# rongzhao-zhang/EfficientQ

Measured on AMD Instinct MI355X. Metric: ptq_calibration_throughput, higher is better.
Workload: dtype i8xi8->i32 (exact) for the Gram systems and per-iteration loss convs of the layers with quantised input, f32/f64 elsewhere

## Files before the change

### efficientq_amd/_lib.py

```python
from __future__ import annotations

import ctypes as C
import os

import torch

_HERE = os.path.dirname(os.path.abspath(__file__))
LIB_PATH = os.path.join(_HERE, "libeffq_hip.so")

EFFQ_OK = 0
_ERR_NAMES = {1: "EFFQ_ERR_ARG", 2: "EFFQ_ERR_HIP", 3: "EFFQ_ERR_WORKSPACE", 4: "EFFQ_ERR_NO_DEVICE",
              5: "EFFQ_ERR_NOT_CONVERGED"}


class EffqError(RuntimeError):
    pass


class Geom(C.Structure):
    _fields_ = [(n, C.c_int32) for n in
                ("N", "C1", "C2", "D", "H", "W", "KD", "KH", "KW", "SD", "SH", "SW", "PD", "PH", "PW")]

    def out_dims(self):
        return ((self.D + 2 * self.PD - self.KD) // self.SD + 1,
# ... 52 lines not shown
    "effq_quant_dequant_f64path": (_I, [_P, _P, _D, _D, _I, _P, _P, _P, _SZ, _P]),
    "effq_reduce_ws_bytes": (_SZ, []),
    "effq_abs_sum_f64": (_I, [_P, _SZ, _P, _P, _P]),
    "effq_moments_f64": (_I, [_P, _SZ, _P, _P, _P]),
    "effq_alpha_stats_f64": (_I, [_P, _P, _D, _D, _I, _SZ, _P, _P, _P, _P]),
    "effq_fp_init": (_I, [_P, _P, _P]),
    "effq_fp_update": (_I, [_P, _D, _I, _P]),
    "effq_alpha_fixed_point": (_I, [_P, _SZ, _I, _D, _D, _D, _I, _I, _P, _P, _P]),
    "effq_fp_small_max": (_SZ, []),
    "effq_fixed_point_small": (_I, [_P, _P, _P, _SZ, _I, _D, _D, _D, _I, _P, _P]),
    "effq_fp_coop_max": (_SZ, []),
    "effq_fp_coop_set_spin_limit": (_I, [C.c_uint]),
    "effq_fixed_point_coop": (_I, [_P, _P, _P, _SZ, _I, _D, _D, _D, _I, _P, _P, _P]),
    "effq_fp_bucket_max": (_SZ, []),
    "effq_fp_bucket_ws_bytes": (_SZ, [_SZ]),
    "effq_fixed_point_bucket": (_I, [_P, _P, _P, _SZ, _I, _D, _D, _D, _I, _P, _P, _SZ, _P]),
    "effq_fp_bracket_ws_bytes": (_SZ, [_SZ]),
    "effq_fp_bracket_init": (_I, [_P, _P, _SZ, _I, _I, _P, _SZ, _P]),
    "effq_fp_bracket_run": (_I, [_P, _SZ, _I, _D, _D, _D, _I, _I, _P, _P, _P]),
    "effq_fp_bracket_stats": (_I, [_P, _SZ, _I, _D, _D, _P, _P, _P]),
    "effq_fp_bracket_update": (_I, [_SZ, _I, _D, _D, _D, _I, _P, _P, _P]),
    "effq_fp_traj_max": (_SZ, []),
    "effq_fp_traj_ws_bytes": (_SZ, [_SZ]),
    "effq_spd_inverse_prepare": (_I, [_P]),
    "effq_fp_traj_pred_bytes": (_SZ, []),
    "effq_fixed_point_traj": (_I, [_P, _P, _P, _SZ, _I, _D, _D, _D, _I, _P, _P, _P, _SZ, _P]),
    "effq_fixed_point_bucket_rec": (_I, [_P, _P, _P, _SZ, _I, _D, _D, _D, _I, _P, _P, _SZ, _P, _P]),
    "effq_fixed_point_coop_rec": (_I, [_P, _P, _P, _SZ, _I, _D, _D, _D, _I, _P, _P, _P, _P]),
    "effq_fp_check": (_I, [_P, _P, _P]),
    "effq_fp_channels_max_row": (_I, []),
    "effq_fixed_point_channels": (_I, [_P, _P, _P, _I, _I, _I, _D, _I, _P, _P, _P, _P]),
    "effq_fixed_point_channels_proj": (_I, [_P, _P, _P, _I, _I, _I, _D, _I, _P, _P, _P, _P, _F, _P, _P, _P, _I, _I, _D,
                                            _D, _P]),
    "effq_gram_packed_elems": (_SZ, [_I, _I]),
    "effq_gram_pack": (_I, [_P, _P, _I, _I, _P, _P]),
    "effq_gram_unpack": (_I, [_P, _I, _I, _P, _P, _P]),
    "effq_act_quant_backward": (_I, [_P, _P, _I, _P, _P, _P, _SZ, _P, _P]),
    "effq_att_classes_ws_bytes": (_SZ, []),
    "effq_att_classes": (_I, [_P, _LL, _P, _P, _P, C.POINTER(C.c_int32), _P, _P]),
    "effq_prof_enable": (_I, [_I]),
    "effq_prof_count": (_I, []),
    "effq_prof_read": (_I, [_I, C.POINTER(ProfRecord)]),
    "effq_admm_num_inverses": (_I, [_D, _D, _I, _I]),
    "effq_admm_run": (_I, [C.POINTER(AdmmRunArgs)]),
    "effq_admm_select_best": (_I, [_P, _I, _P, _P, _SZ, _SZ, _P, _P, _P, _P]),
    "effq_gram_ws_bytes": (_SZ, [_GP, _I]),
    "effq_gram_accum": (_I, [_P, _P, _P, _GP, _I, _P, _P, _I, _P, _SZ, _P]),
    "effq_gram_plan_query": (_I, [_GP, _I, _IP, _IP, _IP, _IP, _LLP, _IP, _IP]),
    "effq_gram_i8_supported": (_I, [_GP, _I]),
    "effq_gram_i8_ws_bytes": (_SZ, [_GP, _I]),
    "effq_gram_accum_i8": (_I, [_P, _P, _GP, _I, _P, _I, _P, _P, _P, _I, _LL, _P, _P, _I, _P, _SZ, _P]),
    "effq_gram_accum_i8_unw": (_I, [_P, _P, _GP, _I, _P, _I, _P, _P, _P, _I, _LL, _P, _P, _I, _P, _P, _P, _SZ, _P]),
    "effq_gram_i8_plan_query": (_I, [_GP, _I, _LL, _IP, _IP, _IP, _IP, _IP, _IP]),
    "effq_upsample_trilinear": (_I, [_P, _I, _I, _I, _I, _I, _I, _I, _I, _P, _P]),
    "effq_gram_f64_supported": (_I, [_GP, _I]),
    "effq_gram_f64_ws_bytes": (_SZ, [_GP, _I]),
    "effq_gram_f64": (_I, [_P, _P, _GP, _I, _P, _P, _P, _SZ, _P]),
    "effq_gram_f64_plan_query": (_I, [_GP, _I, _IP, _IP, _IP, _IP]),
    "effq_gram_f64_pipelined": (_I, [_P, _P, _GP, _I]),
    "effq_gram_loss_ws_bytes": (_SZ, [_I]),
    "effq_gram_loss": (_I, [_P, _P, _P, _P, _P, _I, _I, _I, _P, _P, _SZ, _P]),
    "effq_packed_bytes": (_SZ, [_SZ, _I]),
    "effq_pack_levels": (_I, [_P, _SZ, _I, _P, _P]),
    "effq_unpack_levels": (_I, [_P, _SZ, _I, _P, _P]),
    "effq_ainv_ld": (_I, [_I]),
    "effq_fp_bracket_export_words": (_SZ, []),
    "effq_fp_bracket_export": (_I, [_P, _SZ, _P, _P, _SZ, _P]),
    "effq_fp_bracket_rebase": (_I, [_P, _P, _SZ, _P]),
    "effq_fp_bracket_import": (_I, [_P, _SZ, _P, _I, _SZ, _P, _P, _SZ, _P]),
    "effq_admm_uses_traj": (_I, [_SZ, _I]),
    "effq_gram_loss_i8_supported": (_I, [_I, _I, _I, _I]),
    "effq_gram_loss_i8_num_planes": (_I, [C.c_longlong]),
    "effq_gram_loss_i8_planes_bytes": (_SZ, [_I, _I, _I]),
    "effq_gram_loss_i8_prepare": (_I, [_P, _I, _I, _P, _I, _I, _P, _P, _P]),
    "effq_gram_loss_i8_ws_bytes": (_SZ, []),
    "effq_gram_loss_i8": (_I, [_P, _I, _P, _P, _P, _P, _P, _P, _P, _I, _I, _I, _I, _I, _I, _P, _P, _SZ, _P]),
    "effq_spd_inverse_ws_bytes": (_SZ, [_I]),
    "effq_spd_inverse": (_I, [_P, _I, _I, _D, _D, _P, _P, _SZ, _P]),
    "effq_spd_inverse_plan": (_I, [_I, _IP, _IP, _IP]),
    "effq_prox_plan_query": (_I, [_I, _I, _IP, _IP, _IP, _IP]),
    "effq_prox_ws_bytes": (_SZ, [_I, _I]),
    "effq_prox_solve": (_I, [_P, _P, _P, _P, _P, _P, _I, _I, _I, _D, _D, _P, _P, _P, _SZ, _P]),
    "effq_prox_solve_shifted": (_I, [_P, _P, _P, _P, _P, _P, _I, _I, _I, _D, _D, _D, _I, _P, _P, _P, _SZ, _P]),
    "effq_admm_presum": (_I, [_P, _P, _P, _SZ, _P]),
    "effq_admm_project_dual": (_I, [_P, _P, _P, _I, _P, _P, _F, _P, _SZ, _P]),
    "effq_conv_plan_query": (_I, [_GP, _I, _IP, _IP, _IP, _IP, _IP, _IP, _IP, _IP, _LLP]),
    "effq_conv_i8_plan_query": (_I, [_GP, _I, _IP, _IP, _IP, _IP]),
    "effq_conv_i8s_plan_query": (_I, [_GP, _I, _I, _IP, _IP, _IP, _IP, _IP, _IP, _IP]),
    "effq_conv_i8_supported": (_I, [_GP, _I, _I]),
    "effq_conv_i8s_supported": (_I, [_GP, _I, _I]),
    "effq_conv_i8s_ws_bytes": (_SZ, [_GP, _I, _I]),
    "conv3d_calib_step_i8s": (_I, [_P, _P, _P, _P, _GP, _P, _I, _P, _I, _I, _P, _P, _SZ, _P]),
    "effq_conv_i8_ws_bytes": (_SZ, [_GP]),
    "conv3d_calib_step_i8": (_I, [_P, _P, _P, _P, _GP, _P, _I, _P, _I, _P, _P, _SZ, _P]),
    "effq_conv_i8_out_supported": (_I, [_GP, _I, _I]),
    "conv3d_quant_forward_i8": (_I, [_P, _P, _P, _P, _P, _GP, _P, _I, _P, _I, _P, _P, _P, _SZ, _P]),
    "effq_conv_ws_bytes": (_SZ, [_GP]),
    "conv3d_quant_calib_step": (_I, [_P, _P, _P, _P, _P, _GP, _P, _I, _P, _P, _P, _SZ, _P]),
    "effq_adam_step": (_I, [_P, _P, _P, _P, _D, _D, _D, _D, _I, _SZ, _P]),
    "effq_window_gather": (_I, [_P, _I, _I, _I, _I, _I, _I, _I, _I, _I, _I, _I, _I, _I, _I, _P, _P]),
    "effq_window_put": (_I, [_P, _I, _I, _I, _I, _I, _I, _I, _P, _P]),
    "effq_window_stitch": (_I, [_P, _I, _I, _I, _I, _I, _I, _I, _I, _I, _I, _I, _P, _P, _P, _I, _P, _P]),
    "effq_seg_tallies": (_I, [_P, _P, _I, _LL, _I, _I, _F, _P, _P, _SZ, _P]),
    "effq_seg_sweep": (_I, [_P, _P, _I, _LL, _I, _I, _F, _P, _P]),
    "effq_seg_sweep_edges": (_I, [_I, _F, _P]),
    "effq_seg_sweep_plan": (_I, [_I, _LL, _I, _IP, _IP]),
# ... 73 lines not shown
```

### efficientq_amd/csrc/gram_i8.hip

```cpp
#include <stdint.h>
#include <stdlib.h>
#include "common.h"

namespace effq {

typedef int gi_v4i __attribute__((ext_vector_type(4)));
typedef int gi_v16i __attribute__((ext_vector_type(16)));

constexpr int GI_KC = 128;
constexpr int GI_MB = 128;
constexpr int GI_RS = GI_KC + 16;
constexpr int GI_T = 256;
constexpr int GI_PANEL = GI_MB * GI_RS;
constexpr int GI_LDS = 4 * GI_PANEL + 2 * GI_KC * 16;
constexpr int GI_MAXCLS = 16;
constexpr int GI_MAX_CPS = 1000;

struct GramI8Params {
  const uint8_t* x;
  const int8_t* yd;
  const int* vox_list;
  const int* chunk_cls;
  const int* vtab;
  int N, C1, C2, C2P, D, H, W, OD, OH, OW;
  int KD, KH, KW, SD, SH, SW, PD, PH, PW;
  int T, RX, YR0, E, NB, NBX, npairs;
  long long V;
  int nchunks, nsplit, cps, ncls;
  long long* slabs;
  int debug;
};

__device__ __forceinline__ void gi_transpose4(int r0, int r1, int r2, int r3, int (&o)[4]) {
  const int t0 = __builtin_amdgcn_perm(r1, r0, 0x05010400);
  const int t1 = __builtin_amdgcn_perm(r1, r0, 0x07030602);
  const int t2 = __builtin_amdgcn_perm(r3, r2, 0x05010400);
  const int t3 = __builtin_amdgcn_perm(r3, r2, 0x07030602);
  o[0] = __builtin_amdgcn_perm(t2, t0, 0x05040100);
  o[1] = __builtin_amdgcn_perm(t2, t0, 0x07060302);
  o[2] = __builtin_amdgcn_perm(t3, t1, 0x05040100);
  o[3] = __builtin_amdgcn_perm(t3, t1, 0x07060302);
}

__device__ __forceinline__ gi_v4i gi_build_entry(const GramI8Params& p, int v) {
  gi_v4i e = {0, 0, 0, 0};
  if (v < 0) return e;
  int t = v;
  const int ow = t % p.OW;
  t /= p.OW;
  const int oh = t % p.OH;
  t /= p.OH;
  const int od = t % p.OD;
  const int n = t / p.OD;
  const int id0 = od * p.SD - p.PD, ih0 = oh * p.SH - p.PH, iw0 = ow * p.SW - p.PW;
  unsigned m = 0x80000000u;
  int tap = 0;
  for (int kd = 0; kd < p.KD; ++kd)
    for (int kh = 0; kh < p.KH; ++kh)
      for (int kw = 0; kw < p.KW; ++kw, ++tap) {
        const int id = id0 + kd, ih = ih0 + kh, iw = iw0 + kw;
        const bool ok = id >= 0 && id < p.D && ih >= 0 && ih < p.H && iw >= 0 && iw < p.W;
        m |= (ok ? 1u : 0u) << tap;
      }
  e[0] = ((n * p.D + id0) * p.H + ih0) * p.W + iw0;
  e[1] = (int)m;
  e[2] = v;
  return e;
}

__global__ __launch_bounds__(256) void k_gi_voxtable(GramI8Params p, gi_v4i* __restrict__ table) {
  const long long nslots = (long long)p.nchunks * GI_KC;
  const long long stride = (long long)gridDim.x * blockDim.x;
  for (long long s = (long long)blockIdx.x * blockDim.x + threadIdx.x; s < nslots; s += stride) {
    const int v = (p.vox_list != nullptr) ? p.vox_list[s] : ((s < p.V) ? (int)s : -1);
    table[s] = gi_build_entry(p, v);
  }
}

__global__ __launch_bounds__(GI_T, 2) void k_gram_i8(GramI8Params p) {
  extern __shared__ __attribute__((aligned(16))) unsigned char gi_smem[];
  unsigned char* const panI = gi_smem;
  unsigned char* const panJ = gi_smem + 2 * GI_PANEL;
  gi_v4i* const tbl = reinterpret_cast<gi_v4i*>(gi_smem + 4 * GI_PANEL);

  const int tid = threadIdx.x, lane = tid & 63, wid = tid >> 6;
  const int li = lane & 31, lh = lane >> 5;
  const int wr = wid >> 1, wc = wid & 1;

  int I = 0, rem = blockIdx.x;
  while (rem >= p.NB - I) {
    rem -= p.NB - I;
    ++I;
  }
  const int J = I + rem;
  const bool diag = (I == J);

  const int c_begin = blockIdx.y * p.cps;
  const int c_end = min(c_begin + p.cps, p.nchunks);
  if (c_begin >= c_end) return;

  const int vg = tid & 31, rg = tid >> 5;
  int kindI, tapI, offI, kindJ, tapJ, offJ;
  auto make_rg = [&](int r0, int& kind, int& tap, int& off) {
    kind = 3;
    tap = 0;
    off = 0;
    if (r0 < p.RX) {
      kind = 0;
      tap = r0 / p.C1;
      const int c0 = r0 - tap * p.C1;
      const int kw = tap % p.KW, t2 = tap / p.KW;
      const int kh = t2 % p.KH, kd = t2 / p.KH;
      off = ((kd * p.H + kh) * p.W + kw) * p.C1 + c0;
    } else if (r0 == p.RX) {
      kind = 2;
    } else if (r0 >= p.YR0 && r0 < p.E) {
      kind = 1;
      off = r0 - p.YR0;
    }
  };
  make_rg(I * GI_MB + 16 * rg, kindI, tapI, offI);
  make_rg(J * GI_MB + 16 * rg, kindJ, tapJ, offJ);
  const unsigned char* const srcI = (kindI == 1) ? reinterpret_cast<const unsigned char*>(p.yd) : p.x;
  const unsigned char* const srcJ = (kindJ == 1) ? reinterpret_cast<const unsigned char*>(p.yd) : p.x;
  const int ystride = 4 * p.C2P;

  const gi_v4i* const vtab = reinterpret_cast<const gi_v4i*>(p.vtab);

  gi_v4i vI[4], vJ[4];
  unsigned okI = 0, okJ = 0;
#define GI_FETCH(val, okb, kind, tap, off, src, slot)                                            \
  {                                                                                              \
    okb = 0;                                                                                     \
    _Pragma("unroll") for (int q = 0; q < 4; ++q) {                                              \
      const gi_v4i e = tbl[(slot) * GI_KC + vg + 32 * q];                                        \
      const unsigned m = (unsigned)e[1];                                                         \
      const unsigned okx = (m >> (tap)) & 1u, okv = m >> 31;                                     \
      const unsigned ok = (kind == 0) ? okx : ((kind <= 2) ? okv : 0u);                          \
      const int ax = okx ? (e[0] * p.C1 + (off)) : 0;                                            \
      const int ay = e[2] * ystride + (off);                                                     \
      const int addr = (kind == 0) ? ax : ((kind == 1) ? ay : 0);                                \
      val[q] = *reinterpret_cast<const gi_v4i*>(src + ((EFFQ_DBG(p) == 2) ? 0 : addr));             \
      okb |= ok << q;                                                                            \
    }                                                                                            \
  }
  auto stage = [&](unsigned char* P, gi_v4i (&val)[4], unsigned okb, int kind) {
#pragma unroll
    for (int q = 0; q < 4; ++q) {
      const bool ok = (okb >> q) & 1u;
      gi_v4i z = {0, 0, 0, 0};
      if (kind == 2) z[0] = 1;
      if (!ok || kind >= 2) val[q] = ok ? z : gi_v4i{0, 0, 0, 0};
    }
#pragma unroll
    for (int k = 0; k < 4; ++k) {
      int o[4];
      gi_transpose4(val[0][k], val[1][k], val[2][k], val[3][k], o);
#pragma unroll
      for (int b = 0; b < 4; ++b) *reinterpret_cast<int*>(P + (16 * rg + 4 * k + b) * GI_RS + 4 * vg) = o[b];
    }
  };

  gi_v16i acc[2][2];
#pragma unroll
  for (int m = 0; m < 2; ++m)
#pragma unroll
    for (int n = 0; n < 2; ++n)
#pragma unroll
      for (int r = 0; r < 16; ++r) acc[m][n][r] = 0;
  const bool live = (I * GI_MB + wr * 64 < p.E) && (J * GI_MB + wc * 64 < p.E);

  auto flush = [&](int cls) {
    long long* S = p.slabs + ((size_t)cls * p.npairs + blockIdx.x) * (size_t)(GI_MB * GI_MB);
#pragma unroll
    for (int m = 0; m < 2; ++m)
#pragma unroll
      for (int n = 0; n < 2; ++n)
#pragma unroll
        for (int r = 0; r < 16; ++r) {
          const int row = wr * 64 + m * 32 + (r & 3) + 8 * (r >> 2) + 4 * lh;
          const int col = wc * 64 + n * 32 + li;
          const int v = acc[m][n][r];
          if (v != 0)
            atomicAdd(reinterpret_cast<unsigned long long*>(&S[row * GI_MB + col]), (unsigned long long)(long long)v);
          acc[m][n][r] = 0;
        }
  };

  {
    const int k = tid & (GI_KC - 1);
    const int cc = (tid < GI_KC) ? c_begin : min(c_begin + 1, c_end - 1);
    tbl[(tid < GI_KC ? 0 : 1) * GI_KC + k] = vtab[(size_t)cc * GI_KC + k];
  }
  __syncthreads();
  GI_FETCH(vI, okI, kindI, tapI, offI, srcI, 0)
  if (!diag) GI_FETCH(vJ, okJ, kindJ, tapJ, offJ, srcJ, 0)
  stage(panI, vI, okI, kindI);
  if (!diag) stage(panJ, vJ, okJ, kindJ);
  __syncthreads();

  const bool has_cls = p.chunk_cls != nullptr;
  const int* const clsp = has_cls ? p.chunk_cls : reinterpret_cast<const int*>(p.x);
  int cls_cur = has_cls ? clsp[c_begin] : 0;
  int cls_next = (c_begin + 1 < c_end) ? (has_cls ? clsp[c_begin + 1] : 0) : -1;
  for (int c = c_begin; c < c_end; ++c) {
    const int b = (c - c_begin) & 1;
    const int c2 = min(c + 2, c_end - 1);
    const int cls_raw = clsp[has_cls ? c2 : 0];
    const gi_v4i traw = vtab[(size_t)c2 * GI_KC + (tid & (GI_KC - 1))];
    GI_FETCH(vI, okI, kindI, tapI, offI, srcI, b ^ 1)
    if (!diag) GI_FETCH(vJ, okJ, kindJ, tapJ, offJ, srcJ, b ^ 1)
    __builtin_amdgcn_sched_barrier(0);
    if (live && EFFQ_DBG(p) != 1) {
      const unsigned char* PI = panI + b * GI_PANEL + (wr * 64 + li) * GI_RS + lh * 16;
      const unsigned char* PJ = (diag ? panI : panJ) + b * GI_PANEL + (wc * 64 + li) * GI_RS + lh * 16;
#pragma unroll
      for (int s = 0; s < GI_KC / 32; ++s) {
        gi_v4i a[2], bb[2];
#pragma unroll
        for (int m = 0; m < 2; ++m) a[m] = *reinterpret_cast<const gi_v4i*>(PI + m * 32 * GI_RS + s * 32);
#pragma unroll
        for (int n = 0; n < 2; ++n) bb[n] = *reinterpret_cast<const gi_v4i*>(PJ + n * 32 * GI_RS + s * 32);
#pragma unroll
        for (int m = 0; m < 2; ++m)
#pragma unroll
          for (int n = 0; n < 2; ++n) acc[m][n] = __builtin_amdgcn_mfma_i32_32x32x32_i8(a[m], bb[n], acc[m][n], 0, 0, 0);
      }
    }
    if (cls_next != cls_cur && live) flush(cls_cur);
    if (tid < GI_KC) tbl[b * GI_KC + tid] = traw;
    if (EFFQ_DBG(p) != 3) {
      stage(panI + (b ^ 1) * GI_PANEL, vI, okI, kindI);
      if (!diag) stage(panJ + (b ^ 1) * GI_PANEL, vJ, okJ, kindJ);
    }
    cls_cur = cls_next;
    cls_next = (c + 2 < c_end) ? (has_cls ? cls_raw : 0) : -1;
    __syncthreads();
  }
#undef GI_FETCH
}

__global__ __launch_bounds__(256) void k_gi_absmax(const float* __restrict__ y, size_t n, unsigned* __restrict__ out) {
  float m = 0.0f;
  const size_t stride = (size_t)gridDim.x * blockDim.x;
  for (size_t e = (size_t)blockIdx.x * blockDim.x + threadIdx.x; e < n; e += stride) m = fmaxf(m, fabsf(y[e]));
#pragma unroll
  for (int o = 32; o > 0; o >>= 1) m = fmaxf(m, __shfl_xor(m, o));
  if ((threadIdx.x & 63) == 0) atomicMax(out, __float_as_uint(m));
}

__device__ __forceinline__ int gi_y_exponent(unsigned ymax_bits) {
  const float ymax = __uint_as_float(ymax_bits);
  int ex = 0;
  if (ymax > 0.0f && ymax < 3.0e38f) (void)frexpf(ymax, &ex);
  return ex < -90 ? -90 : ex;
}

__global__ __launch_bounds__(256) void k_gi_ydigits(const float* __restrict__ y, long long V, int C2, int C2P,
                                                    const unsigned* __restrict__ ymax_bits, int8_t* __restrict__ yd) {
  const int ex = gi_y_exponent(*ymax_bits);
  const float scale = ldexpf(1.0f, 30 - ex);
  const size_t tot = (size_t)V * C2P, stride = (size_t)gridDim.x * blockDim.x;
  for (size_t e = (size_t)blockIdx.x * blockDim.x + threadIdx.x; e < tot; e += stride) {
    const size_t v = e / C2P;
    const int c = (int)(e - v * C2P);
    int d[4] = {0, 0, 0, 0};
    if (c < C2) {
      float f = y[v * C2 + c] * scale;
      if (!(fabsf(f) < 1.1e9f)) f = 0.0f;
      int t = (int)rintf(f);
#pragma unroll
      for (int k = 0; k < 3; ++k) {
        d[k] = ((t + 128) & 255) - 128;
        t = (t - d[k]) >> 8;
      }
      d[3] = t;
    }
    int8_t* dst = yd + v * (size_t)(4 * C2P) + c;
#pragma unroll
    for (int k = 0; k < 4; ++k) dst[(size_t)k * C2P] = (int8_t)d[k];
  }
}

__global__ __launch_bounds__(256) void k_gram_i8_finish(GramI8Params p, int n, int hb, const float* __restrict__ alpha,
                                                        int act_levels, const unsigned* __restrict__ ymax_bits,
                                                        const float* __restrict__ cls_w, float* __restrict__ A0,
// ... 56 lines not shown
      }
      val = 2.0 * q * (xb ? s : 1.0) * t;
      dst = B0 + f;
      if (Bu != nullptr) {
        const double vu = q * (xb ? s : 1.0) * tu;
        Bu[f] = accumulate ? Bu[f] + vu : vu;
      }
    }
    *dst = accumulate ? (*dst + (float)val) : (float)val;
  }
}

static int gram_i8_plan(const effq_geom* g, int ncls, long long n_list, GramI8Params* pp) {
  EFFQ_CHECK_ARG(g != nullptr);
  EFFQ_CHECK_ARG(g->N > 0 && g->C1 > 0 && g->C2 > 0 && g->D > 0 && g->H > 0 && g->W > 0);
  EFFQ_CHECK_ARG(g->KD >= 1 && g->KH >= 1 && g->KW >= 1 && g->SD >= 1 && g->SH >= 1 && g->SW >= 1);
  EFFQ_CHECK_ARG((g->C1 % 16) == 0 && g->KD * g->KH * g->KW <= 31);
  EFFQ_CHECK_ARG(ncls >= 1 && ncls <= GI_MAXCLS);
  GramI8Params& p = *pp;
  memset(&p, 0, sizeof(p));
  p.N = g->N; p.C1 = g->C1; p.C2 = g->C2; p.D = g->D; p.H = g->H; p.W = g->W;
  p.KD = g->KD; p.KH = g->KH; p.KW = g->KW; p.SD = g->SD; p.SH = g->SH; p.SW = g->SW;
  p.PD = g->PD; p.PH = g->PH; p.PW = g->PW;
  p.OD = (g->D + 2 * g->PD - g->KD) / g->SD + 1;
  p.OH = (g->H + 2 * g->PH - g->KH) / g->SH + 1;
  p.OW = (g->W + 2 * g->PW - g->KW) / g->SW + 1;
  EFFQ_CHECK_ARG(p.OD > 0 && p.OH > 0 && p.OW > 0);
  p.C2P = (g->C2 + 15) / 16 * 16;
  p.T = p.KD * p.KH * p.KW;
  p.RX = p.T * p.C1;
  p.YR0 = p.RX + 16;
  p.E = p.YR0 + 4 * p.C2P;
  p.NB = (p.E + GI_MB - 1) / GI_MB;
  p.NBX = (p.YR0 + GI_MB - 1) / GI_MB;
  p.npairs = p.NBX * p.NB - p.NBX * (p.NBX - 1) / 2;
  p.V = (long long)p.N * p.OD * p.OH * p.OW;
  EFFQ_CHECK_ARG((long long)g->N * g->D * g->H * g->W * g->C1 < (1ll << 31));
  EFFQ_CHECK_ARG(p.V * 4 * p.C2P < (1ll << 31));
  const long long nchunks = (n_list > 0) ? n_list / GI_KC : (p.V + GI_KC - 1) / GI_KC;
  EFFQ_CHECK_ARG(nchunks > 0 && nchunks < (1ll << 24));
  p.nchunks = (int)nchunks;
  p.ncls = ncls;
  long long want = (3072 + p.npairs - 1) / p.npairs;
  if (want > nchunks / 4) want = nchunks / 4;
  if (want < 1) want = 1;
  long long cps = (nchunks + want - 1) / want;
  if (cps > GI_MAX_CPS) cps = GI_MAX_CPS;
  p.cps = (int)cps;
  p.nsplit = (int)((nchunks + cps - 1) / cps);
  EFFQ_CHECK_ARG(p.nsplit <= 65535);
  return EFFQ_OK;
}

static size_t gram_i8_table_bytes(long long V, int ncls) { return (size_t)(V + (long long)GI_KC * (ncls + 1)) * 16; }

static size_t gram_i8_slab_bytes(const GramI8Params& p) {
  return (size_t)p.ncls * p.npairs * (size_t)(GI_MB * GI_MB) * sizeof(long long);
}

}

using namespace effq;

extern "C" {

int effq_gram_i8_supported(const effq_geom* g, int act_levels) {
  if (g == nullptr) return 0;
  if ((g->C1 % 16) != 0 || g->KD * g->KH * g->KW > 31 || g->KD < 1 || g->KH < 1 || g->KW < 1) return 0;
  if (act_levels < 2 || act_levels > 128) return 0;
  GramI8Params p;
  if (gram_i8_plan(g, 1, 0, &p) != EFFQ_OK) return 0;
  return 1;
}

size_t effq_gram_i8_ws_bytes(const effq_geom* g, int ncls) {
  GramI8Params p;
  if (gram_i8_plan(g, ncls, 0, &p) != EFFQ_OK) return 0;
  return 256 + gram_i8_slab_bytes(p) + (size_t)p.V * 4 * p.C2P + 256 + gram_i8_table_bytes(p.V, ncls) + 256;
}

int effq_gram_accum_i8_unw(const uint8_t* xidx_ndhwc, const float* y_ndhwc, const effq_geom* g, int has_bias,
                           const float* act_alpha_dev, int act_levels, const int32_t* vox_list, const int32_t* chunk_cls,
                           const float* cls_w_dev, int ncls, long long n_list, float* A0, float* B0, int accumulate,
                           double* Au, double* Bu, void* ws, size_t ws_bytes, void* stream) {
  EFFQ_CHECK_ARG((Au == nullptr) == (Bu == nullptr));
  EFFQ_CHECK_ARG(xidx_ndhwc && y_ndhwc && g && act_alpha_dev && A0 && B0 && ws);
  EFFQ_CHECK_ARG(effq_gram_i8_supported(g, act_levels));
  if (vox_list == nullptr) {
    EFFQ_CHECK_ARG(ncls == 1 && chunk_cls == nullptr && n_list == 0);
  } else {
    EFFQ_CHECK_ARG(chunk_cls != nullptr && cls_w_dev != nullptr && n_list > 0 && (n_list % GI_KC) == 0);
  }
  GramI8Params p;
  int rc = gram_i8_plan(g, ncls, n_list, &p);
  if (rc != EFFQ_OK) return rc;
  const size_t slab_bytes = gram_i8_slab_bytes(p);
  const size_t need = 256 + slab_bytes + (size_t)p.V * 4 * p.C2P + 256 + gram_i8_table_bytes(p.V, ncls) + 256;
  EFFQ_CHECK_ARG((size_t)p.nchunks * GI_KC * 16 <= gram_i8_table_bytes(p.V, ncls));
  if (ws_bytes < need) {
    set_error("gram_i8: workspace %zu < required %zu", ws_bytes, need);
    return EFFQ_ERR_WORKSPACE;
  }
  char* base = reinterpret_cast<char*>(ws);
  unsigned* ymax = reinterpret_cast<unsigned*>(base);
  p.slabs = reinterpret_cast<long long*>(base + 256);
  int8_t* yd = reinterpret_cast<int8_t*>(base + 256 + slab_bytes);
  gi_v4i* vtab = reinterpret_cast<gi_v4i*>((reinterpret_cast<uintptr_t>(base + 256 + slab_bytes + (size_t)p.V * 4 * p.C2P) + 255) & ~(uintptr_t)255);
  p.x = xidx_ndhwc;
  p.yd = yd;
  p.vox_list = vox_list;
  p.chunk_cls = chunk_cls;
  p.vtab = reinterpret_cast<const int*>(vtab);
  p.debug = effq_ablate_env("EFFQ_GI8_DEBUG");
  hipStream_t st = as_stream(stream);
  EFFQ_HIP(hipMemsetAsync(base, 0, 256 + slab_bytes, st));
  const size_t ny = (size_t)p.V * p.C2;
  {
    size_t nb = (ny + 255) / 256;
    if (nb > 2048) nb = 2048;
    hipLaunchKernelGGL(k_gi_absmax, dim3((unsigned)nb), dim3(256), 0, st, y_ndhwc, ny, ymax);
    size_t nd = ((size_t)p.V * p.C2P + 255) / 256;
    if (nd > 8192) nd = 8192;
    hipLaunchKernelGGL(k_gi_ydigits, dim3((unsigned)nd), dim3(256), 0, st, y_ndhwc, p.V, p.C2, p.C2P, ymax, yd);
    EFFQ_LAUNCH_CHECK();
  }
  {
    size_t nt = ((size_t)p.nchunks * GI_KC + 255) / 256;
    if (nt > 4096) nt = 4096;
    hipLaunchKernelGGL(k_gi_voxtable, dim3((unsigned)nt), dim3(256), 0, st, p, vtab);
    EFFQ_LAUNCH_CHECK();
  }
  EFFQ_HIP(raise_lds_limit<k_gram_i8>(GI_LDS));
  hipLaunchKernelGGL(k_gram_i8, dim3((unsigned)p.npairs, (unsigned)p.nsplit), dim3(GI_T), GI_LDS, st, p);
  EFFQ_LAUNCH_CHECK();
  const int n = p.RX + (has_bias ? 1 : 0);
  size_t tot = (size_t)n * n + (size_t)p.C2 * n;
  size_t nb = (tot + 255) / 256;
  if (nb > 8192) nb = 8192;
  hipLaunchKernelGGL(k_gram_i8_finish, dim3((unsigned)nb), dim3(256), 0, st, p, n, has_bias ? 1 : 0, act_alpha_dev,
                     act_levels, ymax, cls_w_dev, A0, B0, accumulate, Au, Bu);
  EFFQ_LAUNCH_CHECK();
  return EFFQ_OK;
}

int effq_gram_i8_plan_query(const effq_geom* g, int ncls, long long n_list, int* nb, int* nbx, int* npairs, int* nchunks,
                            int* cps, int* nsplit) {
  EFFQ_CHECK_ARG(nb && nbx && npairs && nchunks && cps && nsplit && n_list >= 0 && (n_list % GI_KC) == 0);
  GramI8Params p;
  const int rc = gram_i8_plan(g, ncls, n_list, &p);
  if (rc != EFFQ_OK) return rc;
  *nb = p.NB;
  *nbx = p.NBX;
  *npairs = p.npairs;
  *nchunks = p.nchunks;
  *cps = p.cps;
  *nsplit = p.nsplit;
  return EFFQ_OK;
}

int effq_gram_accum_i8(const uint8_t* xidx_ndhwc, const float* y_ndhwc, const effq_geom* g, int has_bias,
                       const float* act_alpha_dev, int act_levels, const int32_t* vox_list, const int32_t* chunk_cls,
                       const float* cls_w_dev, int ncls, long long n_list, float* A0, float* B0, int accumulate,
                       void* ws, size_t ws_bytes, void* stream) {
  return effq_gram_accum_i8_unw(xidx_ndhwc, y_ndhwc, g, has_bias, act_alpha_dev, act_levels, vox_list, chunk_cls,
                                cls_w_dev, ncls, n_list, A0, B0, accumulate, nullptr, nullptr, ws, ws_bytes, stream);
}

}

namespace effq {
constexpr int CLS_SLOTS = 32;
constexpr int CLS_MAX = 16;
struct ClsTable {
  unsigned key[CLS_SLOTS];
  unsigned cnt[CLS_SLOTS];
  unsigned cursor[CLS_MAX];
  int overflow;
  int ncls;
  int n_list;
  int slot_cls[CLS_SLOTS];
  unsigned seg_start[CLS_MAX];
  float cls_w[CLS_MAX];
};

__device__ __forceinline__ int cls_find_or_insert(unsigned* keys, unsigned k) {
  unsigned h = (k * 2654435761u) >> 27;
  for (int probe = 0; probe < CLS_SLOTS; ++probe) {
    const unsigned cur = atomicCAS(&keys[h], 0xffffffffu, k);
    if (cur == 0xffffffffu || cur == k) return (int)h;
    h = (h + 1) & (CLS_SLOTS - 1);
  }
  return -1;
}

__global__ __launch_bounds__(256) void k_cls_count(const float* __restrict__ att, long long V, ClsTable* t) {
  __shared__ unsigned lkey[CLS_SLOTS], lcnt[CLS_SLOTS];
  __shared__ int lover;
  if (threadIdx.x < CLS_SLOTS) {
    lkey[threadIdx.x] = 0xffffffffu;
    lcnt[threadIdx.x] = 0u;
  }
  if (threadIdx.x == 0) lover = 0;
  __syncthreads();
  const long long stride = (long long)gridDim.x * blockDim.x;
  for (long long i = (long long)blockIdx.x * blockDim.x + threadIdx.x; i < V; i += stride) {
    const unsigned k = __float_as_uint(att[i]);
    const int sidx = (k == 0xffffffffu) ? -1 : cls_find_or_insert(lkey, k);
    if (sidx < 0)
      lover = 1;
// ... 112 lines not shown
```

### efficientq_amd/hip_ops.py

```python
from __future__ import annotations

import ctypes as C
import math
from typing import Optional, Tuple

import torch

from . import _lib
from ._lib import Geom, check

ADMM_TOL = 1e-5
FP_BRACKET_MIN = 1 << 18
DP_GATHER_AFTER = 4
DP_GATHER_MAX_BYTES = 128 << 20


def _ptr(t: Optional[torch.Tensor]):
    return None if t is None else C.c_void_p(t.data_ptr())


def to_ndhwc(x: torch.Tensor) -> torch.Tensor:
    return x.permute(0, 2, 3, 4, 1).contiguous()


# ... 337 lines not shown
                                                 100 * levels, _ptr(state), _ptr(self._red_ws), _ptr(pred), self.stream),
              "effq_fixed_point_coop_rec")

    @staticmethod
    def read_fp_pred(pred: torch.Tensor):
        i32 = pred[:16].view(torch.int32).cpu()
        f = pred[16:16 + 8 * 40].view(torch.float64).cpu()
        i64 = pred[16 + 8 * 40:16 + 8 * 45].view(torch.int64).cpu()
        fn = pred[16 + 8 * 45:16 + 8 * 53].view(torch.float64).cpu()
        j64 = pred[16 + 8 * 53:16 + 8 * 63].view(torch.int64).cpu()
        K = int(i32[0])
        return {"K": K, "e": int(i32[1]), "lo": f[0:8].tolist(), "hi": f[8:16].tolist(), "eps": f[16:24].tolist(),
                "eps_n": fn.tolist(), "calls": int(i64[0]), "warm_iters": int(i64[1]), "full_iters": int(i64[2]),
                "listed": int(i64[3]), "list_max": int(i64[4]), "ring_iters": int(j64[0]), "ring_listed": int(j64[1]),
                "trace_us": [(int(j64[2 + k]) - int(j64[2])) / 100.0 for k in range(5)],
                "mean_us_phase1_setup_loop": [int(j64[7 + k]) / 100.0 / max(int(i64[0]), 1) for k in range(3)]}

    def fp_check(self, state, err_flag):
        check(self.lib.effq_fp_check(_ptr(state), _ptr(err_flag), self.stream), "effq_fp_check")

    def gram(self, x_ndhwc: torch.Tensor, att: Optional[torch.Tensor], y_ndhwc: torch.Tensor, geom: Geom,
             has_bias: bool, A0: Optional[torch.Tensor] = None, B0: Optional[torch.Tensor] = None):
        x = self._f32(x_ndhwc)
        y = self._f32(y_ndhwc)
        a = self._f32(att) if att is not None else None
        _check_shapes(geom, x, y=y, att=a)
        n = geom.C1 * geom.KD * geom.KH * geom.KW + int(has_bias)
        acc = int(A0 is not None)
        if A0 is not None and (tuple(A0.shape) != (n, n) or tuple(B0.shape) != (geom.C2, n)):
            raise _lib.EffqError("gram: A0/B0 shapes do not match the geometry")
        if A0 is None:
            A0 = torch.empty(n, n, dtype=torch.float32, device=self.device)
            B0 = torch.empty(geom.C2, n, dtype=torch.float32, device=self.device)
        need = self.lib.effq_gram_ws_bytes(C.byref(geom), int(has_bias))
        ws = self._workspace("gram", need)
        check(self.lib.effq_gram_accum(_ptr(x), _ptr(a), _ptr(y), C.byref(geom), int(has_bias), _ptr(A0), _ptr(B0),
                                       acc, _ptr(ws), ws.numel(), self.stream), "effq_gram_accum")
        return A0, B0

    def gram_plan(self, geom: Geom, has_bias: bool) -> dict:
        vec, nb, npairs, nsplit, fold, fin = (C.c_int() for _ in range(6))
        vps = C.c_longlong()
        check(self.lib.effq_gram_plan_query(C.byref(geom), int(has_bias), C.byref(vec), C.byref(nb), C.byref(npairs),
                                            C.byref(nsplit), C.byref(vps), C.byref(fold), C.byref(fin)),
              "effq_gram_plan_query")
        return dict(vec=bool(vec.value), NB=nb.value, npairs=npairs.value, nsplit=nsplit.value, vox_per_split=vps.value,
                    fold=fold.value, finish_blocks=fin.value)

    def gram_i8_plan(self, geom: Geom, ncls: int = 1, n_list: int = 0) -> dict:
        out = [C.c_int() for _ in range(6)]
        check(self.lib.effq_gram_i8_plan_query(C.byref(geom), int(ncls), int(n_list), *[C.byref(o) for o in out]),
              "effq_gram_i8_plan_query")
        return dict(zip(("NB", "NBX", "npairs", "nchunks", "cps", "nsplit"), (o.value for o in out)))

    def gram_f64_plan(self, geom: Geom, has_bias: bool) -> dict:
        out = [C.c_int() for _ in range(4)]
        check(self.lib.effq_gram_f64_plan_query(C.byref(geom), int(has_bias), *[C.byref(o) for o in out]),
              "effq_gram_f64_plan_query")
        return dict(zip(("nchunk", "grid", "ntiles", "tpw"), (o.value for o in out)))

    def gram_i8_supported(self, geom: Geom, act_levels: int) -> bool:
        return bool(self.lib.effq_gram_i8_supported(C.byref(geom), int(act_levels)))

    GRAM_I8_MAX_CLASSES = 16

    def att_classes(self, att: Optional[torch.Tensor]):
        if att is None:
            return (None, None, None, 1)
        key = (att.data_ptr(), att.numel(), att._version)
        hit = self._att_cache.get(key)
        if hit is not None:
            return hit[1]
        flat = self._f32(att).reshape(-1)
        V = flat.numel()
        lst = torch.empty(V + 128 * self.GRAM_I8_MAX_CLASSES, dtype=torch.int32, device=flat.device)
        chunk_cls = torch.empty(V // 128 + self.GRAM_I8_MAX_CLASSES, dtype=torch.int32, device=flat.device)
        cls_w = torch.empty(self.GRAM_I8_MAX_CLASSES, dtype=torch.float32, device=flat.device)
        info = (C.c_int32 * 3)()
        ws = self._workspace("att_cls", self.lib.effq_att_classes_ws_bytes())
        check(self.lib.effq_att_classes(_ptr(flat), V, _ptr(lst), _ptr(chunk_cls), _ptr(cls_w), info, _ptr(ws),
                                        self.stream), "effq_att_classes")
        k, n_list, overflow = int(info[0]), int(info[1]), int(info[2])
        res = None if overflow else (lst[:n_list], chunk_cls[: n_list // 128], cls_w[:k], k)
        if len(self._att_cache) > 16:
            self._att_cache.clear()
        self._att_cache[key] = (att, res)
        return res

    def gram_i8(self, xidx_ndhwc: torch.Tensor, att_cls, y_ndhwc: torch.Tensor, geom: Geom, has_bias: bool,
                act_alpha: torch.Tensor, act_levels: int, A0: Optional[torch.Tensor] = None,
                B0: Optional[torch.Tensor] = None, unweighted: bool = False):
        if xidx_ndhwc.dtype != torch.uint8 or not xidx_ndhwc.is_contiguous():
            raise _lib.EffqError("gram_i8 wants contiguous uint8 level ids")
        y = self._f32(y_ndhwc)
        _check_shapes(geom, xidx_ndhwc, y=y)
        lst, chunk_cls, cls_w, ncls = att_cls
        if lst is not None:
            od, oh, ow = geom.out_dims()
            if (int(lst.numel()) < geom.N * od * oh * ow or lst.numel() % 128 or
                    chunk_cls.numel() * 128 != lst.numel() or cls_w.numel() != ncls):
                raise _lib.EffqError("gram_i8: voxel list does not match the output volume")
        n = geom.C1 * geom.KD * geom.KH * geom.KW + int(has_bias)
        acc = int(A0 is not None)
        if A0 is not None and (tuple(A0.shape) != (n, n) or tuple(B0.shape) != (geom.C2, n)):
            raise _lib.EffqError("gram_i8: A0/B0 shapes do not match the geometry")
        if A0 is None:
# ... 1105 lines not shown
```

### include/effq_hip.h

```cpp
#ifndef EFFQ_HIP_H
#define EFFQ_HIP_H

#include <stddef.h>
#include <stdint.h>

#ifdef __cplusplus
extern "C" {
#endif

enum {
  EFFQ_OK = 0,
  EFFQ_ERR_ARG = 1,
  EFFQ_ERR_HIP = 2,
  EFFQ_ERR_WORKSPACE = 3,
  EFFQ_ERR_NO_DEVICE = 4,
  EFFQ_ERR_NOT_CONVERGED = 5
};

typedef struct effq_geom {
  int32_t N, C1, C2;
  int32_t D, H, W;
  int32_t KD, KH, KW;
  int32_t SD, SH, SW;
  int32_t PD, PH, PW;
// ... 50 lines not shown
size_t effq_fp_traj_pred_bytes(void);
int effq_fixed_point_traj(const float* a, const float* b, float* v_out, size_t n, int levels, double lo, double hi,
                          double tol, int max_iter, effq_fp_state* state_dev, void* pred_dev, void* ws, size_t ws_bytes,
                          void* stream);
int effq_fixed_point_bucket_rec(const float* a, const float* b, float* v_out, size_t n, int levels, double lo, double hi,
                                double tol, int max_iter, effq_fp_state* state_dev, void* ws, size_t ws_bytes,
                                void* pred_dev, void* stream);
int effq_fixed_point_coop_rec(const float* a, const float* b, float* v_out, size_t n, int levels, double lo, double hi,
                              double tol, int max_iter, effq_fp_state* state_dev, void* ws, void* pred_dev, void* stream);

size_t effq_fp_bracket_ws_bytes(size_t n);
int effq_fp_bracket_init(effq_fp_state* state_dev, const double* abs_sums_dev, size_t n, int levels, int list_first,
                         void* ws, size_t ws_bytes, void* stream);
int effq_fp_bracket_run(const float* x, size_t n, int levels, double lo, double hi, double tol, int max_iter, int n_iters,
                        effq_fp_state* state_dev, void* ws, void* stream);
int effq_fp_bracket_stats(const float* x, size_t n, int levels, double lo, double hi, effq_fp_state* state_dev, void* ws,
                          void* stream);
int effq_fp_bracket_update(size_t n, int levels, double lo, double hi, double tol, int max_iter,
                           effq_fp_state* state_dev, void* ws, void* stream);
size_t effq_fp_bracket_export_words(void);
int effq_fp_bracket_export(const void* ws, size_t n, long long* out, float* list_out, size_t list_cap, void* stream);
int effq_fp_bracket_import(const void* ws_src, size_t n_src, const long long* pack_dev, int world, size_t list_cap,
                           effq_fp_state* state_dev, void* ws_dst, size_t ws_dst_bytes, void* stream);
int effq_fp_bracket_rebase(effq_fp_state* state_dev, void* ws, size_t n, void* stream);
int effq_fp_channels_max_row(void);
int effq_fixed_point_channels(const float* a, const float* b, float* v_out, int c2, int nwrow, int levels, double tol,
                              int max_iter, double* alpha_out, int32_t* iters_out, int32_t* err_flag_dev, void* stream);
int effq_fixed_point_channels_proj(const float* wstar, float* dual, float* v_out, int c2, int nwrow, int levels,
                                   double tol, int max_iter, double* alpha_out, int32_t* iters_out, int32_t* err_flag_dev,
                                   float* G, float dual_div, float* Bm, const float* B0, const float* W0, int n, int ldb,
                                   double rho_next, double eta, void* stream);

int effq_fp_check(const effq_fp_state* state_dev, int32_t* err_flag_dev, void* stream);

size_t effq_gram_ws_bytes(const effq_geom* g, int has_bias);
int effq_gram_accum(const float* x_ndhwc, const float* att, const float* y_ndhwc, const effq_geom* g,
                    int has_bias, float* A0, float* B0, int accumulate, void* ws, size_t ws_bytes,
                    void* stream);
int effq_gram_plan_query(const effq_geom* g, int has_bias, int* vec, int* nb, int* npairs, int* nsplit,
                         long long* vox_per_split, int* fold, int* finish_blocks);

int effq_gram_i8_supported(const effq_geom* g, int act_levels);
size_t effq_gram_i8_ws_bytes(const effq_geom* g, int ncls);
int effq_gram_accum_i8(const uint8_t* xidx_ndhwc, const float* y_ndhwc, const effq_geom* g, int has_bias,
                       const float* act_alpha_dev, int act_levels, const int32_t* vox_list,
                       const int32_t* chunk_cls, const float* cls_w_dev, int ncls, long long n_list,
                       float* A0, float* B0, int accumulate, void* ws, size_t ws_bytes, void* stream);
int effq_gram_accum_i8_unw(const uint8_t* xidx_ndhwc, const float* y_ndhwc, const effq_geom* g, int has_bias,
                           const float* act_alpha_dev, int act_levels, const int32_t* vox_list, const int32_t* chunk_cls,
                           const float* cls_w_dev, int ncls, long long n_list, float* A0, float* B0, int accumulate,
                           double* Au, double* Bu, void* ws, size_t ws_bytes, void* stream);
int effq_gram_i8_plan_query(const effq_geom* g, int ncls, long long n_list, int* nb, int* nbx, int* npairs, int* nchunks,
                            int* cps, int* nsplit);

int effq_gram_f64_supported(const effq_geom* g, int has_bias);
size_t effq_gram_f64_ws_bytes(const effq_geom* g, int has_bias);
int effq_gram_f64(const float* x_ndhwc, const float* y_ndhwc, const effq_geom* g, int has_bias, double* Au, double* Bu,
                  void* ws, size_t ws_bytes, void* stream);
int effq_gram_f64_plan_query(const effq_geom* g, int has_bias, int* nchunk, int* grid, int* ntiles, int* tpw);
int effq_gram_f64_pipelined(const float* x_ndhwc, const float* y_ndhwc, const effq_geom* g, int has_bias);

size_t effq_gram_loss_ws_bytes(int n);
int effq_gram_loss(const double* Au, const double* Bu, const double* syy_dev, const float* G, const float* b, int c2, int n,
                   int has_bias, double* sqerr_out, void* ws, size_t ws_bytes, void* stream);

int effq_gram_loss_i8_supported(int c2, int n, int has_bias, int w_levels);
int effq_gram_loss_i8_num_planes(long long kmax);
size_t effq_gram_loss_i8_planes_bytes(int n, int has_bias, int nplanes);
int effq_gram_loss_i8_prepare(const double* Au, int n, int has_bias, const float* act_alpha_dev, int act_levels,
                              int nplanes, int8_t* planes, int32_t* err_flag_dev, void* stream);
size_t effq_gram_loss_i8_ws_bytes(void);
int effq_gram_loss_i8(const int8_t* planes, int nplanes, const double* Au, const double* Bu, const double* syy_dev,
                      const int8_t* Gq, const float* b, const effq_fp_state* states, const float* act_alpha_dev,
                      int act_levels, int w_levels, int c2, int n, int has_bias, int count, double* hist_out, void* ws,
                      size_t ws_bytes, void* stream);


size_t effq_att_classes_ws_bytes(void);
int effq_att_classes(const float* att, long long V, int32_t* vox_list, int32_t* chunk_cls, float* cls_w_dev,
                     int32_t* info_host_out, void* ws, void* stream);

int effq_spd_inverse_prepare(void* stream);
int effq_ainv_ld(int n);
size_t effq_spd_inverse_ws_bytes(int n);
int effq_spd_inverse(const float* A0, int n, int has_bias, double rho, double eta, float* Ainv,
                     void* ws, size_t ws_bytes, void* stream);
int effq_spd_inverse_plan(int n, int* wide, int* nblk, int* pivot_blocks);

size_t effq_prox_ws_bytes(int c2, int n);
int effq_prox_solve(const float* B0, const float* Ainv, const float* W0, const float* b0, const float* G,
                    const float* dual, int c2, int n, int has_bias, double rho, double eta, float* wstar,
                    float* bstar, void* ws, size_t ws_bytes, void* stream);
int effq_prox_plan_query(int c2, int n, int* variant, int* gx, int* gy, int* nsplit);

int effq_prox_solve_shifted(const float* B0, const float* Ainv, const float* W0, const float* b0, const float* G,
                            const float* dual, int c2, int n, int has_bias, double rho, double eta,
                            double rho_inv, int nterms, float* wstar, float* bstar, void* ws, size_t ws_bytes,
                            void* stream);

int effq_admm_presum(const float* wstar, const float* dual, float* v, size_t n, void* stream);
int effq_admm_project_dual(const float* v, const float* wstar, const effq_fp_state* state_dev, int levels,
                           float* G, float* dual, float dual_div, int8_t* Gq_out, size_t n, void* stream);
size_t effq_conv_ws_bytes(const effq_geom* g);
int conv3d_quant_calib_step(const float* xq_ndhwc, const float* G, const float* bias, const float* y_fp,
                            const float* att, const effq_geom* g, const float* act_alpha_dev, int act_levels,
                            double* sqerr_out, float* out, void* ws, size_t ws_bytes, void* stream);
// ... 186 lines not shown
```

Baseline: 25.23.

## Group 2x2 Gram tile pairs per block and sub-split chunk ranges

The int8 Gram kernel is templated on a group size G. With G=2, one 512-thread block computes a 2x2 group of 128x128 tile pairs, and each wave holds a 128x64 accumulator. Every staged I/J panel now feeds two output tiles instead of one, roughly halving global gathers and LDS staging per MFMA. Each split's chunk range is also divided into sub parts to keep the grid large enough. In exchange, LDS use rises to about 150KB per block, which limits residency to one block per CU, and accumulator register pressure doubles. Lower-triangle tiles inside diagonal groups are left idle, and a host override plus a query API are added.

```diff
diff --git a/efficientq_amd/_lib.py b/efficientq_amd/_lib.py
--- a/efficientq_amd/_lib.py
+++ b/efficientq_amd/_lib.py
@@ -128,6 +128,8 @@
     "effq_gram_accum_i8": (_I, [_P, _P, _GP, _I, _P, _I, _P, _P, _P, _I, _LL, _P, _P, _I, _P, _SZ, _P]),
     "effq_gram_accum_i8_unw": (_I, [_P, _P, _GP, _I, _P, _I, _P, _P, _P, _I, _LL, _P, _P, _I, _P, _P, _P, _SZ, _P]),
     "effq_gram_i8_plan_query": (_I, [_GP, _I, _LL, _IP, _IP, _IP, _IP, _IP, _IP]),
+    "effq_gram_i8_group_query": (_I, [_GP, _I, _LL, _IP, _IP, _IP, _IP]),
+    "effq_gram_i8_set_group": (_I, [_I, _I]),
     "effq_upsample_trilinear": (_I, [_P, _I, _I, _I, _I, _I, _I, _I, _I, _P, _P]),
     "effq_gram_f64_supported": (_I, [_GP, _I]),
     "effq_gram_f64_ws_bytes": (_SZ, [_GP, _I]),
diff --git a/efficientq_amd/csrc/gram_i8.hip b/efficientq_amd/csrc/gram_i8.hip
--- a/efficientq_amd/csrc/gram_i8.hip
+++ b/efficientq_amd/csrc/gram_i8.hip
@@ -12,7 +12,9 @@
 constexpr int GI_RS = GI_KC + 16;
 constexpr int GI_T = 256;
 constexpr int GI_PANEL = GI_MB * GI_RS;
-constexpr int GI_LDS = 4 * GI_PANEL + 2 * GI_KC * 16;
+constexpr int GI_GROUP = 2;
+constexpr int gi_lds_bytes(int G) { return 4 * G * GI_PANEL + 2 * GI_KC * 16; }
+static_assert(gi_lds_bytes(GI_GROUP) <= 160 * 1024, "two stages of both group panels and the tables fit one CU's LDS");
 constexpr int GI_MAXCLS = 16;
 constexpr int GI_MAX_CPS = 1000;
 
@@ -27,6 +29,7 @@
   int T, RX, YR0, E, NB, NBX, npairs;
   long long V;
   int nchunks, nsplit, cps, ncls;
+  int sub;
   long long* slabs;
   int debug;
 };
@@ -77,26 +80,36 @@
   }
 }
 
-__global__ __launch_bounds__(GI_T, 2) void k_gram_i8(GramI8Params p) {
+template <int G>
+__global__ __launch_bounds__(G * GI_T, 2) void k_gram_i8(GramI8Params p) {
+  constexpr int GP = G * GI_PANEL;
+  constexpr int MT = 2 * G;
   extern __shared__ __attribute__((aligned(16))) unsigned char gi_smem[];
   unsigned char* const panI = gi_smem;
-  unsigned char* const panJ = gi_smem + 2 * GI_PANEL;
-  gi_v4i* const tbl = reinterpret_cast<gi_v4i*>(gi_smem + 4 * GI_PANEL);
+  unsigned char* const panJ = gi_smem + 2 * GP;
+  gi_v4i* const tbl = reinterpret_cast<gi_v4i*>(gi_smem + 4 * GP);
 
   const int tid = threadIdx.x, lane = tid & 63, wid = tid >> 6;
   const int li = lane & 31, lh = lane >> 5;
-  const int wr = wid >> 1, wc = wid & 1;
-
-  int I = 0, rem = blockIdx.x;
-  while (rem >= p.NB - I) {
-    rem -= p.NB - I;
-    ++I;
-  }
-  const int J = I + rem;
-  const bool diag = (I == J);
-
-  const int c_begin = blockIdx.y * p.cps;
-  const int c_end = min(c_begin + p.cps, p.nchunks);
+  const int wc = wid & 1;
+  const int bi = (G == 2) ? (wid >> 2) : 0, bj = (G == 2) ? ((wid >> 1) & 1) : 0;
+  const int wrow = (G == 2) ? 0 : (wid >> 1) * 64;
+
+  int I0 = 0, rem = blockIdx.x;
+  while (rem >= (p.NB - I0 + G - 1) / G) {
+    rem -= (p.NB - I0 + G - 1) / G;
+    I0 += G;
+  }
+  const int J0 = I0 + rem * G;
+  const bool diag = (I0 == J0);
+  const int I = I0 + bi, J = J0 + bj;
+  const int pair = I * p.NB - I * (I - 1) / 2 + (J - I);
+
+  const int split = blockIdx.y / p.sub, part = blockIdx.y - split * p.sub;
+  const int s_begin = split * p.cps;
+  const int s_len = min(s_begin + p.cps, p.nchunks) - s_begin;
+  const int c_begin = s_begin + s_len * part / p.sub;
+  const int c_end = s_begin + s_len * (part + 1) / p.sub;
   if (c_begin >= c_end) return;
 
   const int vg = tid & 31, rg = tid >> 5;
@@ -119,8 +132,8 @@
       off = r0 - p.YR0;
     }
   };
-  make_rg(I * GI_MB + 16 * rg, kindI, tapI, offI);
-  make_rg(J * GI_MB + 16 * rg, kindJ, tapJ, offJ);
+  make_rg(I0 * GI_MB + 16 * rg, kindI, tapI, offI);
+  make_rg(J0 * GI_MB + 16 * rg, kindJ, tapJ, offJ);
   const unsigned char* const srcI = (kindI == 1) ? reinterpret_cast<const unsigned char*>(p.yd) : p.x;
   const unsigned char* const srcJ = (kindJ == 1) ? reinterpret_cast<const unsigned char*>(p.yd) : p.x;
   const int ystride = 4 * p.C2P;
@@ -161,24 +174,24 @@
     }
   };
 
-  gi_v16i acc[2][2];
-#pragma unroll
-  for (int m = 0; m < 2; ++m)
+  gi_v16i acc[MT][2];
+#pragma unroll
+  for (int m = 0; m < MT; ++m)
 #pragma unroll
     for (int n = 0; n < 2; ++n)
 #pragma unroll
       for (int r = 0; r < 16; ++r) acc[m][n][r] = 0;
-  const bool live = (I * GI_MB + wr * 64 < p.E) && (J * GI_MB + wc * 64 < p.E);
+  const bool live = (I < p.NBX) && (J < p.NB) && (J >= I) && (I * GI_MB + wrow < p.E) && (J * GI_MB + wc * 64 < p.E);
 
   auto flush = [&](int cls) {
-    long long* S = p.slabs + ((size_t)cls * p.npairs + blockIdx.x) * (size_t)(GI_MB * GI_MB);
-#pragma unroll
-    for (int m = 0; m < 2; ++m)
+    long long* S = p.slabs + ((size_t)cls * p.npairs + pair) * (size_t)(GI_MB * GI_MB);
+#pragma unroll
+    for (int m = 0; m < MT; ++m)
 #pragma unroll
       for (int n = 0; n < 2; ++n)
 #pragma unroll
         for (int r = 0; r < 16; ++r) {
-          const int row = wr * 64 + m * 32 + (r & 3) + 8 * (r >> 2) + 4 * lh;
+          const int row = wrow + m * 32 + (r & 3) + 8 * (r >> 2) + 4 * lh;
           const int col = wc * 64 + n * 32 + li;
           const int v = acc[m][n][r];
           if (v != 0)
@@ -190,7 +203,7 @@
   {
     const int k = tid & (GI_KC - 1);
     const int cc = (tid < GI_KC) ? c_begin : min(c_begin + 1, c_end - 1);
-    tbl[(tid < GI_KC ? 0 : 1) * GI_KC + k] = vtab[(size_t)cc * GI_KC + k];
+    if (tid < 2 * GI_KC) tbl[(tid < GI_KC ? 0 : 1) * GI_KC + k] = vtab[(size_t)cc * GI_KC + k];
   }
   __syncthreads();
   GI_FETCH(vI, okI, kindI, tapI, offI, srcI, 0)
@@ -212,17 +225,17 @@
     if (!diag) GI_FETCH(vJ, okJ, kindJ, tapJ, offJ, srcJ, b ^ 1)
     __builtin_amdgcn_sched_barrier(0);
     if (live && EFFQ_DBG(p) != 1) {
-      const unsigned char* PI = panI + b * GI_PANEL + (wr * 64 + li) * GI_RS + lh * 16;
-      const unsigned char* PJ = (diag ? panI : panJ) + b * GI_PANEL + (wc * 64 + li) * GI_RS + lh * 16;
+      const unsigned char* PI = panI + b * GP + (bi * GI_MB + wrow + li) * GI_RS + lh * 16;
+      const unsigned char* PJ = (diag ? panI : panJ) + b * GP + (bj * GI_MB + wc * 64 + li) * GI_RS + lh * 16;
 #pragma unroll
       for (int s = 0; s < GI_KC / 32; ++s) {
-        gi_v4i a[2], bb[2];
-#pragma unroll
-        for (int m = 0; m < 2; ++m) a[m] = *reinterpret_cast<const gi_v4i*>(PI + m * 32 * GI_RS + s * 32);
+        gi_v4i a[MT], bb[2];
+#pragma unroll
+        for (int m = 0; m < MT; ++m) a[m] = *reinterpret_cast<const gi_v4i*>(PI + m * 32 * GI_RS + s * 32);
 #pragma unroll
         for (int n = 0; n < 2; ++n) bb[n] = *reinterpret_cast<const gi_v4i*>(PJ + n * 32 * GI_RS + s * 32);
 #pragma unroll
-        for (int m = 0; m < 2; ++m)
+        for (int m = 0; m < MT; ++m)
 #pragma unroll
           for (int n = 0; n < 2; ++n) acc[m][n] = __builtin_amdgcn_mfma_i32_32x32x32_i8(a[m], bb[n], acc[m][n], 0, 0, 0);
       }
@@ -230,8 +243,8 @@
     if (cls_next != cls_cur && live) flush(cls_cur);
     if (tid < GI_KC) tbl[b * GI_KC + tid] = traw;
     if (EFFQ_DBG(p) != 3) {
-      stage(panI + (b ^ 1) * GI_PANEL, vI, okI, kindI);
-      if (!diag) stage(panJ + (b ^ 1) * GI_PANEL, vJ, okJ, kindJ);
+      stage(panI + (b ^ 1) * GP, vI, okI, kindI);
+      if (!diag) stage(panJ + (b ^ 1) * GP, vJ, okJ, kindJ);
     }
     cls_cur = cls_next;
     cls_next = (c + 2 < c_end) ? (has_cls ? cls_raw : 0) : -1;
@@ -394,6 +407,34 @@
   return EFFQ_OK;
 }
 
+constexpr int GI_GROUP_MIN_CPS = 64;
+static int g_gi_group = 0;
+
+static int gram_i8_group(const GramI8Params& p) {
+  if (g_gi_group != 0) return g_gi_group;
+  return (p.NBX >= 2 && p.cps >= GI_GROUP_MIN_CPS) ? GI_GROUP : 1;
+}
+
+static int gram_i8_sub(const GramI8Params& p, int G) {
+  return (G == GI_GROUP && p.cps >= GI_GROUP_MIN_CPS && 2 * p.nsplit <= 65535) ? 2 : 1;
+}
+
+static int gram_i8_ngroups(const GramI8Params& p, int G) {
+  int n = 0;
+  for (int I0 = 0; I0 < p.NBX; I0 += G) n += (p.NB - I0 + G - 1) / G;
+  return n;
+}
+
+template <int G>
+static hipError_t gram_i8_launch(GramI8Params p, hipStream_t st) {
+  hipError_t e = raise_lds_limit<k_gram_i8<G>>(gi_lds_bytes(G));
+  if (e != hipSuccess) return e;
+  p.sub = gram_i8_sub(p, G);
+  hipLaunchKernelGGL(k_gram_i8<G>, dim3((unsigned)gram_i8_ngroups(p, G), (unsigned)(p.nsplit * p.sub)), dim3(G * GI_T),
+                     gi_lds_bytes(G), st, p);
+  return hipGetLastError();
+}
+
 static size_t gram_i8_table_bytes(long long V, int ncls) { return (size_t)(V + (long long)GI_KC * (ncls + 1)) * 16; }
 
 static size_t gram_i8_slab_bytes(const GramI8Params& p) {
@@ -472,9 +513,7 @@
     hipLaunchKernelGGL(k_gi_voxtable, dim3((unsigned)nt), dim3(256), 0, st, p, vtab);
     EFFQ_LAUNCH_CHECK();
   }
-  EFFQ_HIP(raise_lds_limit<k_gram_i8>(GI_LDS));
-  hipLaunchKernelGGL(k_gram_i8, dim3((unsigned)p.npairs, (unsigned)p.nsplit), dim3(GI_T), GI_LDS, st, p);
-  EFFQ_LAUNCH_CHECK();
+  EFFQ_HIP(gram_i8_group(p) == GI_GROUP ? gram_i8_launch<GI_GROUP>(p, st) : gram_i8_launch<1>(p, st));
   const int n = p.RX + (has_bias ? 1 : 0);
   size_t tot = (size_t)n * n + (size_t)p.C2 * n;
   size_t nb = (tot + 255) / 256;
@@ -497,6 +536,25 @@
   *nchunks = p.nchunks;
   *cps = p.cps;
   *nsplit = p.nsplit;
+  return EFFQ_OK;
+}
+
+int effq_gram_i8_group_query(const effq_geom* g, int ncls, long long n_list, int* gi, int* gj, int* ngroups, int* grid_y) {
+  EFFQ_CHECK_ARG(gi && gj && ngroups && grid_y && n_list >= 0 && (n_list % GI_KC) == 0);
+  GramI8Params p;
+  const int rc = gram_i8_plan(g, ncls, n_list, &p);
+  if (rc != EFFQ_OK) return rc;
+  const int G = gram_i8_group(p);
+  *gi = G;
+  *gj = G;
+  *ngroups = gram_i8_ngroups(p, G);
+  *grid_y = p.nsplit * gram_i8_sub(p, G);
+  return EFFQ_OK;
+}
+
+int effq_gram_i8_set_group(int gi, int gj) {
+  EFFQ_CHECK_ARG(gi == gj && (gi == 0 || gi == 1 || gi == GI_GROUP));
+  g_gi_group = gi;
   return EFFQ_OK;
 }
 
diff --git a/efficientq_amd/hip_ops.py b/efficientq_amd/hip_ops.py
--- a/efficientq_amd/hip_ops.py
+++ b/efficientq_amd/hip_ops.py
@@ -413,6 +413,15 @@
         check(self.lib.effq_gram_i8_plan_query(C.byref(geom), int(ncls), int(n_list), *[C.byref(o) for o in out]),
               "effq_gram_i8_plan_query")
         return dict(zip(("NB", "NBX", "npairs", "nchunks", "cps", "nsplit"), (o.value for o in out)))
+
+    def gram_i8_groups(self, geom: Geom, ncls: int = 1, n_list: int = 0) -> dict:
+        out = [C.c_int() for _ in range(4)]
+        check(self.lib.effq_gram_i8_group_query(C.byref(geom), int(ncls), int(n_list), *[C.byref(o) for o in out]),
+              "effq_gram_i8_group_query")
+        return dict(zip(("gi", "gj", "ngroups", "grid_y"), (o.value for o in out)))
+
+    def gram_i8_set_group(self, gi: int, gj: int) -> None:
+        check(self.lib.effq_gram_i8_set_group(int(gi), int(gj)), "effq_gram_i8_set_group")
 
     def gram_f64_plan(self, geom: Geom, has_bias: bool) -> dict:
         out = [C.c_int() for _ in range(4)]
diff --git a/include/effq_hip.h b/include/effq_hip.h
--- a/include/effq_hip.h
+++ b/include/effq_hip.h
@@ -126,6 +126,8 @@
                            double* Au, double* Bu, void* ws, size_t ws_bytes, void* stream);
 int effq_gram_i8_plan_query(const effq_geom* g, int ncls, long long n_list, int* nb, int* nbx, int* npairs, int* nchunks,
                             int* cps, int* nsplit);
+int effq_gram_i8_group_query(const effq_geom* g, int ncls, long long n_list, int* gi, int* gj, int* ngroups, int* grid_y);
+int effq_gram_i8_set_group(int gi, int gj);
 
 int effq_gram_f64_supported(const effq_geom* g, int has_bias);
 size_t effq_gram_f64_ws_bytes(const effq_geom* g, int has_bias);
```

After: 25.49, median of 6. +1.0%, better.
